# MechaCritter/Python-Visual-Similarity

Measured on AMD Instinct MI355X. Metric: images/sec encoded + top-k retrieved, VLAD K256 RootSIFT, higher is better.
Workload: dtype f32

## Files before the change

include/pvsim.h:

```cpp
#ifndef PVSIM_H
#define PVSIM_H

#include <stddef.h>
#include <stdint.h>

#ifdef __cplusplus
extern "C" {
#endif

#define PVS_VERSION 103

typedef enum {
  PVS_OK = 0,
  PVS_ERR_INVALID = 1,
  PVS_ERR_NO_DEVICE = 2,
  PVS_ERR_OOM = 3,
  PVS_ERR_UNSUPPORTED = 4,
  PVS_ERR_DIM = 5,
  PVS_ERR_CAPACITY = 6
} pvs_status;

typedef enum {
  PVS_DESC_F32 = 0,
  PVS_DESC_F32_ROOTSIFT = 1,
  PVS_DESC_U8_ROOTSIFT = 2
} pvs_desc_kind;

typedef enum {
  PVS_OPT_ASSIGN_PREFILTER = 0,
  PVS_OPT_VLAD_PATH = 1,
  PVS_OPT_TOPK_SELECT_ONLY = 2,
  PVS_OPT_AGG_VARIANT = 3,
  PVS_OPT_FISHER_SCALE = 4,
  PVS_OPT_COUNT_ = 5
} pvs_option;

typedef struct pvs_ctx pvs_ctx;
typedef struct pvs_codebook pvs_codebook;
typedef struct pvs_gmm pvs_gmm;
typedef struct pvs_pca pvs_pca;
typedef struct pvs_comm pvs_comm;

typedef struct {
  double power_norm_weight;
  double norm_order;
  double epsilon;
} pvs_norm_params;

int pvs_version(void);
const char* pvs_last_error(void);
int pvs_device_count(int* count);
int pvs_init(int device_id, void* stream, pvs_ctx** out);
int pvs_destroy(pvs_ctx* ctx);
int pvs_sync(pvs_ctx* ctx);
void* pvs_stream(pvs_ctx* ctx);
int pvs_device_name(pvs_ctx* ctx, char* buf, size_t buflen);
int pvs_set_option(pvs_ctx* ctx, int option, int value);
int pvs_get_option(pvs_ctx* ctx, int option, int* value);

int pvs_malloc(pvs_ctx* ctx, size_t bytes, void** dptr);
int pvs_free(pvs_ctx* ctx, void* dptr);
int pvs_memcpy_h2d(pvs_ctx* ctx, void* dst_dev, const void* src_host, size_t bytes);
int pvs_memcpy_d2h(pvs_ctx* ctx, void* dst_host, const void* src_dev, size_t bytes);
int pvs_memset(pvs_ctx* ctx, void* dst_dev, int value, size_t bytes);

int pvs_fill_dev(pvs_ctx* ctx, void* dst_dev, int64_t n_elems, int elem_bytes, uint64_t pattern);
int pvs_stream_wait(pvs_ctx* waiter, pvs_ctx* signal);

int pvs_codebook_create(pvs_ctx* ctx, const float* centroids , int K, int D, pvs_codebook** out);
int pvs_codebook_destroy(pvs_ctx* ctx, pvs_codebook* cb);
int pvs_gmm_create(pvs_ctx* ctx, const double* weights , const double* means ,
                   const double* covariances , int K, int D, pvs_gmm** out);
int pvs_gmm_destroy(pvs_ctx* ctx, pvs_gmm* g);
int pvs_pca_create(pvs_ctx* ctx, const float* components , const float* mean ,
                   int n_components, int d_in, pvs_pca** out);
int pvs_pca_destroy(pvs_ctx* ctx, pvs_pca* p);

int pvs_vlad_encode(pvs_ctx* ctx, const pvs_codebook* cb, const pvs_pca* pca, const void* desc,
                    int desc_kind, const int64_t* offsets, int64_t n_images, const pvs_norm_params* prm,
                    float* out, int32_t* out_labels);
int pvs_vlad_encode_dev(pvs_ctx* ctx, const pvs_codebook* cb, const pvs_pca* pca, const void* d_desc,
                        int desc_kind, const int64_t* d_offsets, int64_t n_images, int64_t total_desc,
                        const pvs_norm_params* prm, float* d_out, int32_t* d_labels, float* d_inv_norm);
int pvs_kmeans_predict_dev(pvs_ctx* ctx, const pvs_codebook* cb, const void* d_desc, int desc_kind,
                           int64_t total_desc, int32_t* d_labels);

int pvs_fisher_encode(pvs_ctx* ctx, const pvs_gmm* g, const pvs_pca* pca, const void* desc, int desc_kind,
// ... 154 lines not shown
```

python-visual-similarity_amd/csrc/assign_prefilter.hpp:

```cpp
#pragma once

#include "common.hpp"
#include "desc_load.hpp"

namespace pvs {

typedef _Float16 f16x8_t __attribute__((ext_vector_type(8)));
typedef _Float16 f16x4_t __attribute__((ext_vector_type(4)));

constexpr int ASSIGN_THREADS = 512;
constexpr int ASSIGN_ROWS = (ASSIGN_THREADS / 64) * 32;

struct Assign16Args {
  const void* X;
  int64_t total;
  int D, ld;
  const _Float16* C16;
  const float* cnorm;
  int K_pad, D_pad16;
  int c_shift;
  float cmax;
  const _Float16* cnk;
  int cn_e1, K;
  int32_t* labels;
  int64_t* amb_rows;
  unsigned long long* amb_count;
  int64_t cap;
  float2* rowstat;
  unsigned long long* stamps;
  int nprod;
  int shape16;
};

int launch_assign16x(pvs_ctx* ctx, const Assign16Args& p, int kind, size_t lds, int grid);

__device__ __forceinline__ void pf_fill_sqrt_table(uint32_t* lds_t) {
  if (threadIdx.x < 256) {
    const float sv = sqrtf((float)threadIdx.x);
    const _Float16 hi = (_Float16)sv, lo = (_Float16)(sv - (float)hi);
    lds_t[threadIdx.x] = (uint32_t)__builtin_bit_cast(unsigned short, hi) | ((uint32_t)__builtin_bit_cast(unsigned short, lo) << 16);
  }
}
__device__ __forceinline__ void pf_u8_fragment(const uint32_t* lds_t, const uint32_t* xw, f16x8_t* xh, f16x8_t* xl) {
  uint32_t hw[4], lw[4];
#pragma unroll
  for (int i = 0; i < 2; ++i)
#pragma unroll
    for (int pq = 0; pq < 2; ++pq) {
      const uint32_t w = xw[i];
      const uint32_t e0 = lds_t[(w >> (16 * pq)) & 0xffu], e1 = lds_t[(w >> (16 * pq + 8)) & 0xffu];
      hw[2 * i + pq] = __builtin_amdgcn_perm(e1, e0, 0x05040100u);
      lw[2 * i + pq] = __builtin_amdgcn_perm(e1, e0, 0x07060302u);
    }
  *xh = __builtin_bit_cast(f16x8_t, make_uint4(hw[0], hw[1], hw[2], hw[3]));
  *xl = __builtin_bit_cast(f16x8_t, make_uint4(lw[0], lw[1], lw[2], lw[3]));
}

template <int KIND, int NP, bool LUT>
__device__ __forceinline__ float prefilter_eps(float nx, float cmax, float lut_sd, float sqrt_d) {
  const float xc = nx * cmax;
  constexpr float conv_err = DescTraits<KIND>::rootsift ? 4.8e-7f : 0.f;
  const float cc = LUT ? cmax * cmax * lut_sd : cmax * cmax;
  constexpr float drop_err = (3 - NP) * 4.9e-4f;
  return 2.f * (4.8e-7f + 2.4e-7f + 4.8e-5f + 7.7e-6f + 1e-9f + conv_err + drop_err) * xc * (1.f + sqrt_d * 1e-9f) + (LUT ? 6.0e-7f : 2.4e-7f) * (cc + 2.f * xc);
}

__device__ __forceinline__ void pf_label_or_list(const Assign16Args& a, bool settled, bool leader, int64_t row, int bidx, int lane,
                                                 unsigned int* s_count, int64_t* my_rows) {
  const bool amb = leader && !settled;
  const unsigned long long amask = __ballot(amb);
  unsigned int base = 0;
  if (amask != 0ull) {
    if (lane == 0) base = atomicAdd(s_count, (unsigned int)__popcll(amask));
    base = __shfl(base, 0, 64);
  }
  if (leader) {
    if (settled) a.labels[row] = bidx;
    else my_rows[base + __popcll(amask & ((1ull << lane) - 1ull))] = row;
  }
}

}
```

python-visual-similarity_amd/csrc/common.hpp:

```cpp
#pragma once
#include <hip/hip_runtime.h>

#include <cmath>
#include <cstdarg>
#include <cstdint>
#include <cstdio>
#include <cstring>
#include <map>
#include <type_traits>
#include <vector>

#include "../../include/pvsim.h"
#include "../../include/pvsim_diag.h"
#include "workspace.hpp"

#define PVS_EXPORT extern "C" __attribute__((visibility("default")))

namespace pvs {

void set_error(const char* fmt, ...);

#define PVS_FAIL(code, ...)        \
  do {                             \
    ::pvs::set_error(__VA_ARGS__); \
    return (code);                 \
  } while (0)

#define PVS_HIP(expr)                                                                    \
  do {                                                                                   \
    hipError_t e__ = (expr);                                                             \
    if (e__ != hipSuccess) {                                                             \
      ::pvs::set_error("%s failed: %s (%s:%d)", #expr, hipGetErrorString(e__), __FILE__, \
                       __LINE__);                                                        \
      return e__ == hipErrorOutOfMemory ? PVS_ERR_OOM : PVS_ERR_NO_DEVICE;               \
    }                                                                                    \
  } while (0)

#define PVS_TRY(expr)                 \
  do {                                \
    int s__ = (expr);                 \
    if (s__ != PVS_OK) return s__;    \
  } while (0)

constexpr int WAVE = 64;

enum TimerSlot { T_ASSIGN = 0, T_AGGREGATE = 1, T_GEMM = 2, T_TOPK = 3, T_FPOST = 4, T_FMOM = 5, T_MISC = 6, T_RESCORE = 7 };

struct TimerRec {
  hipEvent_t a, b;
  int slot;
};

}

struct pvs_ctx {
  int device = 0;
  hipStream_t stream = nullptr;
  bool owns_stream = false;
  int num_cu = 256;
  static constexpr int NWS = 17;
  void* ws[NWS] = {};
  size_t ws_bytes[NWS] = {};
  struct GemmPlanSlot {
    int key[4] = {-1, -1, -1, -1};
    int n_main = 0, n_tail = 0, splitk = 1;
    void* d_tiles = nullptr;
    size_t cap = 0;
  } gemm_plan[5];
  std::map<const void*, int> lds_attr;
  int opt[PVS_OPT_COUNT_] = {1, 0, 0, 0, 0};
  unsigned int* d_queue = nullptr;
  unsigned long long* d_fused_stamps = nullptr;
  bool timers_on = false;
  std::vector<pvs::TimerRec> pending;
  std::vector<hipEvent_t> event_pool;
  std::multimap<size_t, void*> block_cache;
  std::map<void*, size_t> block_size;
  size_t block_cache_bytes = 0;
  void* h_stage = nullptr;
  size_t h_stage_bytes = 0;
  static constexpr int DSIFT_RING = 4;
  void* dsift_h[DSIFT_RING] = {};
  size_t dsift_h_bytes[DSIFT_RING] = {};
  hipEvent_t dsift_ev[DSIFT_RING] = {};
  int dsift_next = 0;
  double t_total[PVS_TIMER_SLOTS] = {0};
  int64_t t_count[PVS_TIMER_SLOTS] = {0};
};

struct pvs_codebook {
  int K = 0, D = 0;
  int K_pad = 0, D_pad = 0;
  float* d_cent = nullptr;
  float* d_cpad = nullptr;
  float* d_cnorm = nullptr;
  void* d_c16 = nullptr;
  int D_pad16 = 0;
  int c16_shift = 0;
  float cmax = 0.f;
  void* d_cnk = nullptr;
  void* d_c16n = nullptr;
  int cn_e1 = 0;
};

struct pvs_gmm {
  int K = 0, D = 0;
  double* d_w = nullptr;
  double* d_mu = nullptr;
  double* d_cov = nullptr;
  double* d_prec = nullptr;
  double* d_mup = nullptr;
  double* d_inv_mu = nullptr;
  double* d_inv_sg = nullptr;
  double* d_const = nullptr;
};

struct pvs_pca {
  int C = 0, Din = 0;
  float* d_comp = nullptr;
  float* d_off = nullptr;
};

namespace pvs {
// ... 131 lines not shown
```

python-visual-similarity_amd/csrc/vlad.hip:

```cpp
#include "assign_prefilter.hpp"

namespace pvs {

typedef float f32x16 __attribute__((ext_vector_type(16)));

struct AssignArgs {
  const void* X;
  int64_t total;
  int D, ld;
  const float* Cpad;
  const float* cnorm;
  int K_pad, D_pad;
  int32_t* labels;
  const int64_t* rows;
  const unsigned long long* nrows;
  int64_t rows_cap;
};

constexpr int ASSIGN_DCHUNK = 128;

template <int NT, int KIND, bool VEC>
__global__ __launch_bounds__(ASSIGN_THREADS, 2) void assign_kernel(AssignArgs a) {
  extern __shared__ __attribute__((aligned(16))) char smem[];
  constexpr int CB = 32 * NT;
  const int cw_max = a.D_pad < ASSIGN_DCHUNK ? a.D_pad : ASSIGN_DCHUNK;
  const int stride = cw_max + 4;
  float* lds_c = reinterpret_cast<float*>(smem);
  float* lds_n = lds_c + CB * stride;

  const int lane = threadIdx.x & 63, wave = threadIdx.x >> 6;
  const int j = lane & 31, h = lane >> 5;
  const int ncb = a.K_pad / CB;
  const int nsc = (a.D_pad + ASSIGN_DCHUNK - 1) / ASSIGN_DCHUNK;
  const bool restage = (ncb * nsc) > 1;
  const int64_t n_items = a.rows ? (int64_t)a.nrows[blockIdx.x] : a.total;
  const int64_t nblocks = (n_items + ASSIGN_ROWS - 1) / ASSIGN_ROWS;
  const int64_t* const my_rows = a.rows ? a.rows + (int64_t)blockIdx.x * a.rows_cap : nullptr;

  auto stage = [&](int cb, int sc) {
    const int cw = min(ASSIGN_DCHUNK, a.D_pad - sc * ASSIGN_DCHUNK);
    const int c4n = cw >> 2;
    for (int idx = threadIdx.x; idx < CB * c4n; idx += ASSIGN_THREADS) {
      const int r = idx / c4n, c4 = idx - r * c4n;
      const float4 v = *reinterpret_cast<const float4*>(a.Cpad + (int64_t)(cb * CB + r) * a.D_pad +
                                                        sc * ASSIGN_DCHUNK + 4 * c4);
      *reinterpret_cast<float4*>(lds_c + r * stride + 4 * c4) = v;
    }
    for (int idx = threadIdx.x; idx < CB; idx += ASSIGN_THREADS) lds_n[idx] = a.cnorm[cb * CB + idx];
  };

  if (!restage) {
    stage(0, 0);
    __syncthreads();
  }

  for (int64_t blk = my_rows ? 0 : blockIdx.x; blk < nblocks; blk += my_rows ? 1 : gridDim.x) {
    const int64_t item = blk * ASSIGN_ROWS + wave * 32 + j;
    const bool rvalid = item < n_items;
    const int64_t row = (my_rows && rvalid) ? my_rows[item] : item;
    float best = INFINITY;
    int bidx = 0;

    for (int cb = 0; cb < ncb; ++cb) {
      f32x16 acc[NT];
#pragma unroll
      for (int t = 0; t < NT; ++t)
#pragma unroll
        for (int r = 0; r < 16; ++r) acc[t][r] = 0.f;

      for (int sc = 0; sc < nsc; ++sc) {
        if (restage) {
          __syncthreads();
          stage(cb, sc);
          __syncthreads();
        }
        const int dc = sc * ASSIGN_DCHUNK;
        const int nt = min(ASSIGN_DCHUNK, a.D_pad - dc) >> 3;

        float4 xb[16];
#pragma unroll
        for (int t = 0; t < 16; ++t) {
          xb[t] = make_float4(0.f, 0.f, 0.f, 0.f);
          if (t < nt) {
            const int d = dc + 8 * t + 4 * h;
            if constexpr (VEC) {
              if (rvalid && d < a.D) xb[t] = load4<KIND>(a.X, row, a.ld, d);
            } else {
              if (rvalid) {
// ... 406 lines not shown
    }
  }
  __syncthreads();
  if (threadIdx.x == 0) a.amb_count[blockIdx.x] = s_count;
}

template <int NT, int KIND>
static int launch_assign_nt(pvs_ctx* ctx, const AssignArgs& a, bool vec, size_t lds, int grid) {
  auto kv = assign_kernel<NT, KIND, true>;
  auto ks = assign_kernel<NT, KIND, false>;
  return launch_lds(ctx, vec ? kv : ks, dim3(grid), dim3(ASSIGN_THREADS), lds, a);
}

template <int KIND>
static int launch_assign_kind(pvs_ctx* ctx, const AssignArgs& a, int nt, bool vec, size_t lds, int grid) {
  switch (nt) {
    case 8: return launch_assign_nt<8, KIND>(ctx, a, vec, lds, grid);
    case 4: return launch_assign_nt<4, KIND>(ctx, a, vec, lds, grid);
    case 2: return launch_assign_nt<2, KIND>(ctx, a, vec, lds, grid);
    default: return launch_assign_nt<1, KIND>(ctx, a, vec, lds, grid);
  }
}

template <int NT, int KIND>
static int launch_assign16_nt(pvs_ctx* ctx, const Assign16Args& p, bool vec, size_t lds, int grid) {
  auto kv = assign16_kernel<NT, KIND, true, 0>;
  auto ks = assign16_kernel<NT, KIND, false, 0>;
  auto k8 = assign16_kernel<NT, KIND, true, 8>;
  auto k = vec ? (p.D == 128 && p.D_pad16 == 128 ? k8 : kv) : ks;
  if constexpr (NT == 8) {
    if (k == k8 && p.nprod == 3 && p.shape16 && p.stamps == nullptr) return launch_assign16x(ctx, p, KIND, lds, grid);
  }
  if constexpr (NT == 8) {
    if (k == k8 && p.nprod == 2) k = assign16_kernel<NT, KIND, true, 8, false, 2>;
    if (k == k8 && p.nprod == 1) k = assign16_kernel<NT, KIND, true, 8, false, 1>;
  }
  if constexpr (NT == 8) {
    if (p.stamps != nullptr && k == k8) k = assign16_kernel<NT, KIND, true, 8, true>;
  }
  return launch_lds(ctx, k, dim3(grid), dim3(ASSIGN_THREADS), lds, p);
}
template <int KIND>
static int launch_assign16_kind(pvs_ctx* ctx, const Assign16Args& p, int nt, bool vec, size_t lds, int grid) {
  switch (nt) {
    case 8: return launch_assign16_nt<8, KIND>(ctx, p, vec, lds, grid);
    case 4: return launch_assign16_nt<4, KIND>(ctx, p, vec, lds, grid);
    case 2: return launch_assign16_nt<2, KIND>(ctx, p, vec, lds, grid);
    case 1: return launch_assign16_nt<1, KIND>(ctx, p, vec, lds, grid);
    default: PVS_FAIL(PVS_ERR_INVALID, "assignment prefilter: unexpected table padding");
  }
}
static int launch_assign16(pvs_ctx* ctx, const Assign16Args& p, int kind, int nt, bool vec, size_t lds, int grid) {
  return dispatch_desc_kind(kind, [&](auto k) { return launch_assign16_kind<decltype(k)::value>(ctx, p, nt, vec, lds, grid); });
}

int assign_tiles_for(int K) {
  const int k32 = (K + 31) / 32 * 32;
  return k32 > 128 ? 8 : (k32 > 64 ? 4 : (k32 > 32 ? 2 : 1));
}

int launch_assign(pvs_ctx* ctx, const pvs_codebook* cb, const void* d_desc, int kind, int64_t total, int ld,
                  int32_t* d_labels, const float2** rowstat_out) {
  if (rowstat_out) *rowstat_out = nullptr;
  if (total <= 0) return PVS_OK;
  const bool rs = kind != PVS_DESC_F32;
  if (rs && cb->D > ASSIGN_DCHUNK)
    PVS_FAIL(PVS_ERR_UNSUPPORTED, "fused RootSIFT needs D <= %d (got %d)", ASSIGN_DCHUNK, cb->D);
  const int nt = assign_tiles_for(cb->K);
  if (cb->K_pad % (32 * nt) != 0) PVS_FAIL(PVS_ERR_INVALID, "codebook padding does not match the tile count");
  AssignArgs a{d_desc, total, cb->D, ld, cb->d_cpad, cb->d_cnorm, cb->K_pad, cb->D_pad, d_labels, nullptr, nullptr, 0};
  const int esz = kind == PVS_DESC_U8_ROOTSIFT ? 1 : 4;
  const bool vec = (cb->D % 4 == 0) && (ld % 4 == 0) && ((reinterpret_cast<uintptr_t>(d_desc) % (4 * esz)) == 0);
  const int cw = cb->D_pad < ASSIGN_DCHUNK ? cb->D_pad : ASSIGN_DCHUNK;
  const size_t lds = (size_t)(32 * nt) * (cw + 4) * 4 + (size_t)(32 * nt) * 4;
  const int64_t nblocks = (total + ASSIGN_ROWS - 1) / ASSIGN_ROWS;
  const int grid = (int)(nblocks < ctx->num_cu ? nblocks : ctx->num_cu);
  ScopedTimer tm(ctx, T_ASSIGN);
  const bool pre = cb->d_c16 != nullptr && total >= 4096 && ctx->opt[PVS_OPT_ASSIGN_PREFILTER] != 0;
  if (pre) {
    const int64_t cap = (nblocks + grid - 1) / grid * ASSIGN_ROWS;
    char* ws = nullptr;
    const bool stat = rowstat_out != nullptr && kind == PVS_DESC_U8_ROOTSIFT;
    WsLayout<> lay;
    const auto cnt_p = lay.add<unsigned long long>((size_t)grid);
    const auto rows_p = lay.add<int64_t>((size_t)grid * cap);
    const auto stat_p = lay.add<float2>(stat ? (size_t)total : 0);
    PVS_TRY(ws_reserve(ctx, WS_LISTS, lay.bytes(), &ws));
    unsigned long long* cnt = cnt_p(ws);
    int64_t* rows = rows_p(ws);
    float2* rowstat = stat ? stat_p(ws) : nullptr;
    if (stat) *rowstat_out = rowstat;
    Assign16Args p{d_desc, total, cb->D, ld, static_cast<const _Float16*>(cb->d_c16), cb->d_cnorm, cb->K_pad, cb->D_pad16,
                   cb->c16_shift, cb->cmax, static_cast<const _Float16*>(cb->d_cnk), cb->cn_e1, cb->K, d_labels, rows, cnt, cap, rowstat,
                   ctx->d_fused_stamps, ctx->opt[PVS_OPT_ASSIGN_PREFILTER] == 2 ? 2 : (ctx->opt[PVS_OPT_ASSIGN_PREFILTER] == 3 ? 1 : 3),
                   ctx->opt[PVS_OPT_ASSIGN_PREFILTER] == 4 ? 1 : 0};
    const size_t lds16 = (size_t)2 * cb->K_pad * (128 + 8) * 2 + (size_t)cb->K_pad * 4 + (size_t)cb->K_pad * 8 + 1024;
    PVS_TRY(launch_assign16(ctx, p, kind, cb->K_pad / 32, vec, lds16, grid));
    a.rows = rows;
    a.nrows = cnt;
    a.rows_cap = cap;
  }
  return dispatch_desc_kind(kind, [&](auto k) { return launch_assign_kind<decltype(k)::value>(ctx, a, nt, vec, lds, grid); });
}

struct AggArgs {
  const void* X;
  int D, ld;
  const int64_t* offsets;
  const int32_t* labels;
  const float* cent;
  int K;
  float power, eps;
  int norm_mode;
  float norm_p;
  float* out;
  float* inv_norm;
  const float2* rowstat;
};

constexpr int AGG_THREADS = 256;
constexpr int AGG_WAVES = AGG_THREADS / 64;
constexpr int AGG_CHUNK = 4096;

template <int KIND, int GROUP, int VW, int NREG, bool HIOCC = false>
__global__ __launch_bounds__(AGG_THREADS, (HIOCC ? 8 : 1)) void vlad_aggregate_kernel(AggArgs a) {
  extern __shared__ __attribute__((aligned(16))) char smem[];
  const int K = a.K, D = a.D;
  int* hist = reinterpret_cast<int*>(smem);
  int* start = hist + AGG_WAVES * K;
  float* rowsq = reinterpret_cast<float*>(start + K + 1);
  int* scan_tmp = reinterpret_cast<int*>(rowsq + K);
  uint16_t* order = reinterpret_cast<uint16_t*>(scan_tmp + AGG_WAVES);

  const int img = blockIdx.x;
  const int tid = threadIdx.x, lane = tid & 63, wave = tid >> 6;
  const int64_t row0 = a.offsets[img];
  const int64_t n = a.offsets[img + 1] - row0;
  float* out_img = a.out + (int64_t)img * K * D;

  constexpr int NGROUPS = AGG_THREADS / GROUP;
  const int grp = tid / GROUP, gl = tid % GROUP;
  int kbits = 0;
  while ((1 << kbits) < K) ++kbits;

  const int64_t nchunks = n > 0 ? (n + AGG_CHUNK - 1) / AGG_CHUNK : 1;
  for (int64_t ch = 0; ch < nchunks; ++ch) {
    const int64_t cbase = row0 + ch * AGG_CHUNK;
    const int cn = (int)min((int64_t)AGG_CHUNK, n - ch * AGG_CHUNK);
    const bool last = (ch == nchunks - 1);

    for (int i = tid; i < AGG_WAVES * K; i += AGG_THREADS) hist[i] = 0;
    __syncthreads();
    const int per_wave = (cn + AGG_WAVES - 1) / AGG_WAVES;
// ... 467 lines not shown
```

python-visual-similarity_amd/csrc/vlad_fused.hip:

```cpp
#include "common.hpp"
#include "desc_load.hpp"

namespace pvs {

typedef float f32x16 __attribute__((ext_vector_type(16)));
typedef _Float16 f16x8_t __attribute__((ext_vector_type(8)));
typedef _Float16 f16x4_t __attribute__((ext_vector_type(4)));

constexpr int FU_THREADS = 512;
constexpr int FU_R = 64;
constexpr int FU_XS = 132;
constexpr int FU_TS = 1056;
constexpr int FU_TILE = 8 * FU_TS;
constexpr int FU_UNUSABLE = 0x7fffffff;
constexpr int FU_KB = 4;

constexpr int FU_OFF_X32 = 0;
constexpr int FU_OFF_XH = FU_OFF_X32 + FU_R * FU_XS * 4;
constexpr int FU_OFF_XL = FU_OFF_XH + 2 * FU_TILE;
constexpr int FU_OFF_NX = FU_OFF_XL + 2 * FU_TILE;
constexpr int FU_OFF_XSH = FU_OFF_NX + 256;
constexpr int FU_OFF_CAND = FU_OFF_XSH + 256;
constexpr int FU_OFF_ENT = FU_OFF_CAND + 8 * FU_R * 8;
constexpr int FU_OFF_ENTV = FU_OFF_ENT + 2048;
constexpr int FU_OFF_ROWSQ = FU_OFF_ENTV + 4096;
constexpr int FU_OFF_MISC = FU_OFF_ROWSQ + 1024;
constexpr int FU_LDS = FU_OFF_MISC + 64;

struct FusedArgs {
  const void* X;
  int ld;
  const int64_t* offsets;
  int64_t n_images;
  const _Float16* c16n;
  const _Float16* cnk;
  const float* cnorm;
  const float* cent;
  const float* cpad;
  int K, c_shift, cn_e1;
  float cmax;
  float power, eps;
  int norm_mode;
  float norm_p;
  float* out;
  float* inv_norm;
  int32_t* labels;
  unsigned int* queue;
  unsigned long long* stamps;
};

template <int KIND>
struct FuStage {
  float4 v[4];
};
// ... 240 lines not shown
        const float margin = usable ? (eps_a * s_nx[lane] + eps_b) * ldexpf(1.f, a.c_shift + xsh) : 0.f;
        const bool settled = usable && label < a.K && (t1 - t2 > margin);
        const float thr = t1 - margin;
        const unsigned long long umask = __ballot(rvalid && !settled);
        FU_STAMP(2)
        if constexpr (DIAG) { dg_c[0] += 1; dg_c[3] += __popcll(umask); }
        if (umask != 0ull) {
          int cm = 0, am = 0;
          if (rvalid && !settled) {
            if (!usable || label >= a.K) {
              cm = 0xff; am = 0xff;
            } else {
#pragma unroll
              for (int w = 0; w < 8; ++w) {
                const float2 c = s_cand[w * FU_R + lane];
                if (c.x >= thr) cm |= 1 << w;
                if (c.y >= thr) am |= 1 << w;
              }
            }
          }
          const int ne = __popc(cm);
          int incl = ne;
#pragma unroll
          for (int d = 1; d < 64; d <<= 1) {
            const int o = __shfl_up(incl, d, 64);
            if (lane >= d) incl += o;
          }
          const int ebase = incl - ne;
          const int E = __shfl(incl, 63, 64);
          if constexpr (DIAG) { dg_c[1] += 1; dg_c[2] += E; }
          if (wave == 0 && ne > 0) {
            int e = ebase;
            for (int w = 0; w < 8; ++w)
              if (cm & (1 << w)) {
                const int sidx = 31 - (__float_as_int(s_cand[w * FU_R + lane].x) & 31);
                s_ent[e++] = lane | (w << 8) | (((am >> w) & 1) << 12) | (sidx << 16);
              }
          }
          __syncthreads();
          for (int e0 = 0; e0 < E; e0 += 16) {
            const int e = e0 + 2 * wave + h;
            const bool elive = e < E;
            const int ent = elive ? s_ent[e] : 0;
            const int er = ent & 0xff, ew = (ent >> 8) & 7, eall = (ent >> 12) & 1, esi = (ent >> 16) & 31;
            const int k = 32 * ew + (eall ? j : esi);
            const bool active = elive && (eall || j == 0);
            const float* xr = x32 + er * FU_XS;
            const float* cr = a.cpad + (size_t)k * 128;
            float dot = 0.f;
#pragma unroll 2
            for (int b8 = 0; b8 < 128; b8 += 8) {
              const float4 xa = *reinterpret_cast<const float4*>(xr + b8), xb = *reinterpret_cast<const float4*>(xr + b8 + 4);
              const float4 ca = *reinterpret_cast<const float4*>(cr + b8), cb = *reinterpret_cast<const float4*>(cr + b8 + 4);
              dot = fmaf(ca.x, xa.x, dot); dot = fmaf(cb.x, xb.x, dot);
              dot = fmaf(ca.y, xa.y, dot); dot = fmaf(cb.y, xb.y, dot);
              dot = fmaf(ca.z, xa.z, dot); dot = fmaf(cb.z, xb.z, dot);
              dot = fmaf(ca.w, xa.w, dot); dot = fmaf(cb.w, xb.w, dot);
            }
            const float v = fmaf(-2.f, dot, a.cnorm[k]);
            const bool ok = active && (v < INFINITY);
            float vv = ok ? v : INFINITY;
            int kk = ok ? k : 0x7fffffff;
#pragma unroll
            for (int m = 16; m >= 1; m >>= 1) {
              const float ov = __shfl_xor(vv, m, 64);
              const int okk = __shfl_xor(kk, m, 64);
              const bool take = ov < vv || (ov == vv && okk < kk);
              vv = take ? ov : vv;
              kk = take ? okk : kk;
            }
            if (elive && j == 0) s_entv[e] = make_float2(vv, __int_as_float(kk));
          }
          __syncthreads();
          if (rvalid && !settled) {
            float bv = INFINITY;
            int bk = 0x7fffffff;
            for (int i = 0; i < ne; ++i) {
              const float2 r = s_entv[ebase + i];
              const int rk = __float_as_int(r.y);
              if (r.x < bv || (r.x == bv && rk < bk)) { bv = r.x; bk = rk; }
            }
            label = bv < INFINITY ? bk : 0;
          }
        }
        FU_STAMP(3)
        if (a.labels != nullptr && wave == 0 && rvalid) a.labels[sbase + lane] = label;

        unsigned long long mine = __ballot(rvalid && (label >> 5) == wave);
        while (mine != 0ull) {
          int rr[FU_KB], ll[FU_KB];
          int cntb = 0;
#pragma unroll
          for (int u = 0; u < FU_KB; ++u) {
            const bool live = mine != 0ull;
            const int r = live ? (int)__builtin_ctzll(mine) : 0;
            if (live) { mine &= mine - 1ull; ++cntb; }
            rr[u] = r;
            ll[u] = __builtin_amdgcn_readlane(label, r);
          }
          float2 xv[FU_KB], cv[FU_KB];
#pragma unroll
          for (int u = 0; u < FU_KB; ++u) {
            xv[u] = *reinterpret_cast<const float2*>(x32 + rr[u] * FU_XS + 2 * lane);
            cv[u] = *reinterpret_cast<const float2*>(a.cent + (size_t)ll[u] * 128 + 2 * lane);
          }
#pragma unroll
          for (int u = 0; u < FU_KB; ++u) {
            if (u < cntb) {
              const float dx = xv[u].x - cv[u].x, dy = xv[u].y - cv[u].y;
#define FU_ADD(c) case c: acc[2 * c] += dx; acc[2 * c + 1] += dy; break;
// ... 124 lines not shown
```

python-visual-similarity_amd/pvsim/_ffi.py:

```python
from __future__ import annotations

import ctypes as C
import os
import threading

import numpy as np

from ._errors import CapacityError

_HERE = os.path.dirname(os.path.abspath(__file__))
LIB_PATH = os.environ.get("PVSIM_LIB", os.path.join(_HERE, "libpvsim_hip.so"))

PVS_OK, PVS_ERR_INVALID, PVS_ERR_NO_DEVICE, PVS_ERR_OOM, PVS_ERR_UNSUPPORTED, PVS_ERR_DIM, PVS_ERR_CAPACITY = range(7)
_EXC = {PVS_ERR_INVALID: ValueError, PVS_ERR_NO_DEVICE: RuntimeError, PVS_ERR_OOM: MemoryError,
        PVS_ERR_UNSUPPORTED: NotImplementedError, PVS_ERR_DIM: RuntimeError, PVS_ERR_CAPACITY: CapacityError}

DESC_F32, DESC_F32_ROOTSIFT, DESC_U8_ROOTSIFT = 0, 1, 2
OPT_ASSIGN_PREFILTER, OPT_VLAD_PATH, OPT_TOPK_SELECT_ONLY, OPT_AGG_VARIANT, OPT_FISHER_SCALE = 0, 1, 2, 3, 4
PIX_U8_RGB, PIX_U8_GRAY, PIX_F32_RGB, PIX_F32_GRAY = 0, 1, 2, 3
DSIFT_U8, DSIFT_F32, DSIFT_F32_RAW, DSIFT_F32_QUANT = 0, 1, 2, 3
COMBINE_CHUNK_BYTES, COMBINE_BATCH = 8192, 8
VLAD_PATH_AUTO, VLAD_PATH_GATHER, VLAD_PATH_STREAM, VLAD_PATH_FUSED = 0, 1, 2, 3
TIMER_NAMES = ("assign", "aggregate", "cosine_gemm", "topk", "fisher_posterior", "fisher_moments", "misc", "rescore")


class NormParams(C.Structure):
    _fields_ = [("power_norm_weight", C.c_double), ("norm_order", C.c_double), ("epsilon", C.c_double)]


_vp, _i64, _int, _sz = C.c_void_p, C.c_int64, C.c_int, C.c_size_t
_pp = C.POINTER(C.c_void_p)
_np = C.POINTER(NormParams)

SIGNATURES = {
    "pvs_version": [],
    "pvs_last_error": [],
    "pvs_device_count": [C.POINTER(C.c_int)],
    "pvs_init": [_int, _vp, _pp],
    "pvs_destroy": [_vp],
    "pvs_sync": [_vp],
    "pvs_stream": [_vp],
    "pvs_device_name": [_vp, C.c_char_p, _sz],
    "pvs_set_option": [_vp, _int, _int],
    "pvs_get_option": [_vp, _int, C.POINTER(C.c_int)],
    "pvs_malloc": [_vp, _sz, _pp],
    "pvs_free": [_vp, _vp],
    "pvs_memcpy_h2d": [_vp, _vp, _vp, _sz],
    "pvs_memcpy_d2h": [_vp, _vp, _vp, _sz],
    "pvs_memset": [_vp, _vp, _int, _sz],
    "pvs_fill_dev": [_vp, _vp, _i64, _int, C.c_uint64],
    "pvs_stream_wait": [_vp, _vp],
    "pvs_comm_unique_id": [_vp],
    "pvs_comm_init": [_vp, _int, _int, _vp, _pp],
    "pvs_comm_destroy": [_vp],
    "pvs_comm_library": [],
    "pvs_allgather_dev": [_vp, _vp, _vp, _sz],
    "pvs_alltoall_dev": [_vp, _vp, _vp, _sz],
    "pvs_sendrecv_dev": [_vp, _int, _vp, _vp, _vp, _vp, _vp],
    "pvs_allreduce_max_f64": [_vp, _vp, _int],
    "pvs_comm_barrier": [_vp],
    "pvs_codebook_create": [_vp, _vp, _int, _int, _pp],
    "pvs_codebook_destroy": [_vp, _vp],
    "pvs_gmm_create": [_vp, _vp, _vp, _vp, _int, _int, _pp],
    "pvs_gmm_destroy": [_vp, _vp],
    "pvs_pca_create": [_vp, _vp, _vp, _int, _int, _pp],
    "pvs_pca_destroy": [_vp, _vp],
    "pvs_vlad_encode": [_vp, _vp, _vp, _vp, _int, _vp, _i64, _np, _vp, _vp],
    "pvs_vlad_encode_dev": [_vp, _vp, _vp, _vp, _int, _vp, _i64, _i64, _np, _vp, _vp, _vp],
    "pvs_kmeans_predict_dev": [_vp, _vp, _vp, _int, _i64, _vp],
    "pvs_fisher_encode": [_vp, _vp, _vp, _vp, _int, _vp, _i64, _np, _vp],
    "pvs_fisher_encode_dev": [_vp, _vp, _vp, _vp, _int, _vp, _i64, _i64, _np, _vp, _int],
# ... 131 lines not shown
```

Baseline: 416,900.

## Add near-candidate pass to resolve ambiguous assignment rows before full exact assign

New measurement: 418,700, median of 6. About the same (+0.4%).

```diff
diff --git a/include/pvsim.h b/include/pvsim.h
--- a/include/pvsim.h
+++ b/include/pvsim.h
@@ -32,7 +32,8 @@
   PVS_OPT_TOPK_SELECT_ONLY = 2,
   PVS_OPT_AGG_VARIANT = 3,
   PVS_OPT_FISHER_SCALE = 4,
-  PVS_OPT_COUNT_ = 5
+  PVS_OPT_ASSIGN_NEAR = 5,
+  PVS_OPT_COUNT_ = 6
 } pvs_option;
 
 typedef struct pvs_ctx pvs_ctx;
diff --git a/python-visual-similarity_amd/csrc/assign_prefilter.hpp b/python-visual-similarity_amd/csrc/assign_prefilter.hpp
--- a/python-visual-similarity_amd/csrc/assign_prefilter.hpp
+++ b/python-visual-similarity_amd/csrc/assign_prefilter.hpp
@@ -65,6 +65,101 @@
   return 2.f * (4.8e-7f + 2.4e-7f + 4.8e-5f + 7.7e-6f + 1e-9f + conv_err + drop_err) * xc * (1.f + sqrt_d * 1e-9f) + (LUT ? 6.0e-7f : 2.4e-7f) * (cc + 2.f * xc);
 }
 
+template <int KIND>
+struct PfRow {
+  f16x8_t xh[8], xl[8];
+  float nx;
+  float lut_sd = 1.f;
+  _Float16 lut_f1 = (_Float16)0.f, lut_f2 = (_Float16)0.f;
+  int x_shift = 0;
+  bool finite;
+};
+template <int KIND>
+__device__ __forceinline__ void pf_row_front(const Assign16Args& a, int64_t r, int h, const uint32_t* lds_t, PfRow<KIND>& o) {
+  constexpr bool LUT = KIND == PVS_DESC_U8_ROOTSIFT;
+  if constexpr (LUT) {
+    uint32_t xw[8][2];
+    const uint8_t* pr = static_cast<const uint8_t*>(a.X) + r * a.ld + 4 * h;
+#pragma unroll
+    for (int t = 0; t < 8; ++t) {
+      xw[t][0] = *reinterpret_cast<const uint32_t*>(pr + 16 * t);
+      xw[t][1] = *reinterpret_cast<const uint32_t*>(pr + 16 * t + 8);
+    }
+    unsigned ssum = 0;
+#pragma unroll
+    for (int t = 0; t < 8; ++t) {
+      ssum = __builtin_amdgcn_sad_u8(xw[t][0], 0u, ssum);
+      ssum = __builtin_amdgcn_sad_u8(xw[t][1], 0u, ssum);
+    }
+    ssum += __shfl_xor(ssum, 32, 64);
+    const float sf = (float)ssum, dd = sf + 1e-7f;
+    o.lut_sd = sqrtf(dd);
+    const float ff = ldexpf(o.lut_sd, a.cn_e1);
+    o.lut_f1 = (_Float16)ff;
+    o.lut_f2 = (_Float16)(ff - (float)o.lut_f1);
+    o.finite = ff >= 0.125f && ff <= 32768.f;
+    o.nx = sqrtf(sf) * 1.0001f;
+#pragma unroll
+    for (int t = 0; t < 8; ++t) pf_u8_fragment(lds_t, xw[t], &o.xh[t], &o.xl[t]);
+  } else {
+    float xf[8][8];
+#pragma unroll
+    for (int t = 0; t < 8; ++t) {
+      const float4 v0 = load4<KIND>(a.X, r, a.ld, 16 * t + 4 * h);
+      const float4 v1 = load4<KIND>(a.X, r, a.ld, 16 * t + 4 * h + 8);
+      xf[t][0] = v0.x; xf[t][1] = v0.y; xf[t][2] = v0.z; xf[t][3] = v0.w;
+      xf[t][4] = v1.x; xf[t][5] = v1.y; xf[t][6] = v1.z; xf[t][7] = v1.w;
+    }
+    float n2 = 0.f, amax = 0.f, rs_r = 0.f;
+    if constexpr (DescTraits<KIND>::rootsift) {
+      float s = 0.f, rmax = 0.f;
+#pragma unroll
+      for (int t = 0; t < 8; ++t)
+#pragma unroll
+        for (int q = 0; q < 8; ++q) {
+          s += xf[t][q];
+          rmax = fmaxf(rmax, xf[t][q]);
+        }
+      s += __shfl_xor(s, 32, 64);
+      rmax = fmaxf(rmax, __shfl_xor(rmax, 32, 64));
+      rs_r = 1.0f / (s + 1e-7f);
+      n2 = s * rs_r * 1.0001f;
+      amax = __builtin_amdgcn_sqrtf(rmax * rs_r) * 1.0001f;
+      if (!(s >= 0.f) || !(rmax * rs_r <= 3.0e38f)) n2 = NAN;
+    } else {
+#pragma unroll
+      for (int t = 0; t < 8; ++t)
+#pragma unroll
+        for (int q = 0; q < 8; ++q) {
+          n2 = fmaf(xf[t][q], xf[t][q], n2);
+          amax = fmaxf(amax, fabsf(xf[t][q]));
+        }
+      n2 += __shfl_xor(n2, 32, 64);
+      amax = fmaxf(amax, __shfl_xor(amax, 32, 64));
+    }
+    o.nx = sqrtf(n2) * 1.0001f;
+    int ex = 13;
+    if (amax > 0.f) (void)frexpf(amax, &ex);
+    o.x_shift = 13 - ex;
+    o.finite = o.nx <= 3.0e38f;
+    if (o.x_shift > 40 || o.x_shift < -40) { o.finite = false; o.x_shift = 0; }
+    if (o.x_shift + a.cn_e1 < -14 || o.x_shift + a.cn_e1 > 15) o.finite = false;
+    const float xs = ldexpf(1.f, o.x_shift);
+    const float rs_rs = rs_r * xs * xs;
+#pragma unroll
+    for (int t = 0; t < 8; ++t)
+#pragma unroll
+      for (int q = 0; q < 8; ++q) {
+        float v;
+        if constexpr (DescTraits<KIND>::rootsift) v = __builtin_amdgcn_sqrtf(xf[t][q] * rs_rs);
+        else v = xf[t][q] * xs;
+        const _Float16 hi = (_Float16)v;
+        o.xh[t][q] = hi;
+        o.xl[t][q] = (_Float16)(v - (float)hi);
+      }
+  }
+}
+
 __device__ __forceinline__ void pf_label_or_list(const Assign16Args& a, bool settled, bool leader, int64_t row, int bidx, int lane,
                                                  unsigned int* s_count, int64_t* my_rows) {
   const bool amb = leader && !settled;
diff --git a/python-visual-similarity_amd/csrc/common.hpp b/python-visual-similarity_amd/csrc/common.hpp
--- a/python-visual-similarity_amd/csrc/common.hpp
+++ b/python-visual-similarity_amd/csrc/common.hpp
@@ -68,7 +68,7 @@
     size_t cap = 0;
   } gemm_plan[5];
   std::map<const void*, int> lds_attr;
-  int opt[PVS_OPT_COUNT_] = {1, 0, 0, 0, 0};
+  int opt[PVS_OPT_COUNT_] = {1, 0, 0, 0, 0, 0};
   unsigned int* d_queue = nullptr;
   unsigned long long* d_fused_stamps = nullptr;
   bool timers_on = false;
diff --git a/python-visual-similarity_amd/csrc/exact_dot.hpp b/python-visual-similarity_amd/csrc/exact_dot.hpp
--- /dev/null
+++ b/python-visual-similarity_amd/csrc/exact_dot.hpp
@@ -0,0 +1,15 @@
+#pragma once
+
+#include "common.hpp"
+
+namespace pvs {
+
+__device__ __forceinline__ float exact_dot_step8(const float4 ca, const float4 cb, const float4 xa, const float4 xb, float dot) {
+  dot = fmaf(ca.x, xa.x, dot); dot = fmaf(cb.x, xb.x, dot);
+  dot = fmaf(ca.y, xa.y, dot); dot = fmaf(cb.y, xb.y, dot);
+  dot = fmaf(ca.z, xa.z, dot); dot = fmaf(cb.z, xb.z, dot);
+  dot = fmaf(ca.w, xa.w, dot); dot = fmaf(cb.w, xb.w, dot);
+  return dot;
+}
+
+}
diff --git a/python-visual-similarity_amd/csrc/vlad.hip b/python-visual-similarity_amd/csrc/vlad.hip
--- a/python-visual-similarity_amd/csrc/vlad.hip
+++ b/python-visual-similarity_amd/csrc/vlad.hip
@@ -1,4 +1,5 @@
 #include "assign_prefilter.hpp"
+#include "exact_dot.hpp"
 
 namespace pvs {
 
@@ -34,6 +35,7 @@
   const int nsc = (a.D_pad + ASSIGN_DCHUNK - 1) / ASSIGN_DCHUNK;
   const bool restage = (ncb * nsc) > 1;
   const int64_t n_items = a.rows ? (int64_t)a.nrows[blockIdx.x] : a.total;
+  if (a.rows && n_items == 0) return;
   const int64_t nblocks = (n_items + ASSIGN_ROWS - 1) / ASSIGN_ROWS;
   const int64_t* const my_rows = a.rows ? a.rows + (int64_t)blockIdx.x * a.rows_cap : nullptr;
 
@@ -546,6 +548,267 @@
 }
 static int launch_assign16(pvs_ctx* ctx, const Assign16Args& p, int kind, int nt, bool vec, size_t lds, int grid) {
   return dispatch_desc_kind(kind, [&](auto k) { return launch_assign16_kind<decltype(k)::value>(ctx, p, nt, vec, lds, grid); });
+}
+
+constexpr int NEAR_SLOTS = 7;
+
+struct AssignNearArgs {
+  Assign16Args p;
+  const float* Cpad;
+  unsigned long long* cand;
+  int64_t* ovf_rows;
+  unsigned long long* ovf_count;
+  unsigned long long* stats;
+};
+
+constexpr int NEAR_CSTRIDE = 132;
+constexpr size_t NEAR_LDS1 = (size_t)2 * 256 * (128 + 8) * 2 + 256 * 8 + 1024 + (size_t)NEAR_SLOTS * ASSIGN_THREADS * 4;
+constexpr size_t NEAR_LDS2 = (size_t)256 * NEAR_CSTRIDE * 4 + 256 * 4;
+constexpr size_t NEAR_LDS = NEAR_LDS1 > NEAR_LDS2 ? NEAR_LDS1 : NEAR_LDS2;
+
+template <int KIND>
+__global__ __launch_bounds__(ASSIGN_THREADS, 2) void assign_near_kernel(AssignNearArgs a) {
+  extern __shared__ __attribute__((aligned(16))) char smem[];
+  __shared__ unsigned int s_ovf, s_stat[2];
+  const Assign16Args& p = a.p;
+  const int64_t n_items = (int64_t)p.amb_count[blockIdx.x];
+  if (n_items == 0) {
+    if (threadIdx.x == 0) a.ovf_count[blockIdx.x] = 0ull;
+    return;
+  }
+  constexpr bool LUT = KIND == PVS_DESC_U8_ROOTSIFT;
+  constexpr int stride = 128 + 8;
+  _Float16* lds_h = reinterpret_cast<_Float16*>(smem);
+  _Float16* lds_l = lds_h + 256 * stride;
+  _Float16* lds_k = lds_l + 256 * stride;
+  uint32_t* lds_t = reinterpret_cast<uint32_t*>(lds_k + 4 * 256);
+  float* lds_v = reinterpret_cast<float*>(lds_t + 256);
+  const int lane = threadIdx.x & 63, wave = threadIdx.x >> 6;
+  const int j = lane & 31, h = lane >> 5;
+  const int64_t nblocks = (n_items + ASSIGN_ROWS - 1) / ASSIGN_ROWS;
+  const int64_t* const my_rows = p.amb_rows + (int64_t)blockIdx.x * p.cap;
+  unsigned long long* const my_cand = a.cand + (int64_t)blockIdx.x * p.cap;
+  int64_t* const my_ovf = a.ovf_rows + (int64_t)blockIdx.x * p.cap;
+
+  for (int idx = threadIdx.x; idx < 2 * 256 * 16; idx += ASSIGN_THREADS) {
+    const int r = idx >> 4, c8 = idx & 15;
+    *reinterpret_cast<uint4*>(lds_h + r * stride + 8 * c8) = *reinterpret_cast<const uint4*>(p.C16 + (int64_t)r * 128 + 8 * c8);
+  }
+  for (int idx = threadIdx.x; idx < 256; idx += ASSIGN_THREADS)
+    *reinterpret_cast<uint2*>(lds_k + 4 * idx) = *reinterpret_cast<const uint2*>(p.cnk + 4 * idx);
+  if constexpr (LUT) pf_fill_sqrt_table(lds_t);
+  if (threadIdx.x == 0) { s_ovf = 0u; s_stat[0] = 0u; s_stat[1] = 0u; }
+  __syncthreads();
+  const float sqrt_d = sqrtf((float)p.D);
+
+  for (int64_t blk = 0; blk < nblocks; ++blk) {
+    const int64_t item = blk * ASSIGN_ROWS + wave * 32 + j;
+    const bool rvalid = item < n_items;
+    const int64_t row = my_rows[rvalid ? item : n_items - 1];
+    PfRow<KIND> x;
+    pf_row_front<KIND>(p, row, h, lds_t, x);
+    f16x8_t cnb;
+    {
+      const _Float16 pw = (h == 0 && x.finite) ? (_Float16)ldexpf(1.f, x.x_shift + p.cn_e1) : (_Float16)0.f;
+#pragma unroll
+      for (int q = 0; q < 8; ++q) cnb[q] = (_Float16)0.f;
+      if constexpr (LUT) {
+        if (h == 0 && x.finite) { cnb[0] = x.lut_f1; cnb[1] = x.lut_f2; cnb[2] = x.lut_f1; cnb[3] = x.lut_f2; cnb[4] = x.lut_f1; cnb[5] = x.lut_f2; }
+      } else {
+        cnb[0] = pw; cnb[1] = pw; cnb[2] = pw;
+      }
+    }
+    const float m2s = -2.f * ldexpf(1.f, -(x.x_shift + p.c_shift));
+    const float eps2 = 2.f * prefilter_eps<KIND, 3, LUT>(x.nx, p.cmax, x.lut_sd, sqrt_d);
+    float smax = -INFINITY;
+    unsigned long long rpk = 0ull;
+    int rcnt = 0;
+#pragma unroll
+    for (int g = 0; g < 4; ++g) {
+      f32x16 acc[2];
+#pragma unroll
+      for (int u = 0; u < 2; ++u)
+#pragma unroll
+        for (int r = 0; r < 16; ++r) acc[u][r] = 0.f;
+#pragma unroll
+      for (int t = 0; t < 8; ++t) {
+        f16x8_t fh[2], fl[2];
+#pragma unroll
+        for (int u = 0; u < 2; ++u) {
+          fh[u] = *reinterpret_cast<const f16x8_t*>(lds_h + (32 * (2 * g + u) + j) * stride + 16 * t + 8 * h);
+          fl[u] = *reinterpret_cast<const f16x8_t*>(lds_l + (32 * (2 * g + u) + j) * stride + 16 * t + 8 * h);
+        }
+        __builtin_amdgcn_sched_barrier(0);
+#pragma unroll
+        for (int u = 0; u < 2; ++u) acc[u] = __builtin_amdgcn_mfma_f32_32x32x16_f16(fl[u], x.xh[t], acc[u], 0, 0, 0);
+#pragma unroll
+        for (int u = 0; u < 2; ++u) acc[u] = __builtin_amdgcn_mfma_f32_32x32x16_f16(fh[u], x.xl[t], acc[u], 0, 0, 0);
+#pragma unroll
+        for (int u = 0; u < 2; ++u) acc[u] = __builtin_amdgcn_mfma_f32_32x32x16_f16(fh[u], x.xh[t], acc[u], 0, 0, 0);
+        __builtin_amdgcn_sched_barrier(0);
+      }
+#pragma unroll
+      for (int u = 0; u < 2; ++u) {
+        const f16x4_t ck = *reinterpret_cast<const f16x4_t*>(lds_k + 4 * (32 * (2 * g + u) + j));
+        f16x8_t ca;
+#pragma unroll
+        for (int q = 0; q < 8; ++q) ca[q] = (_Float16)0.f;
+        if constexpr (LUT) {
+          if (h == 0) { ca[0] = ck[0]; ca[1] = ck[0]; ca[2] = ck[1]; ca[3] = ck[1]; ca[4] = ck[2]; ca[5] = ck[2]; }
+        } else {
+          if (h == 0) { ca[0] = ck[0]; ca[1] = ck[1]; ca[2] = ck[2]; }
+        }
+        acc[u] = __builtin_amdgcn_mfma_f32_32x32x16_f16(ca, cnb, acc[u], 0, 0, 0);
+      }
+      float gm = -INFINITY;
+#pragma unroll
+      for (int u = 0; u < 2; ++u)
+#pragma unroll
+        for (int r = 0; r < 16; ++r) gm = fmaxf(gm, acc[u][r]);
+      gm = fmaxf(gm, __shfl_xor(gm, 32, 64));
+      smax = fmaxf(smax, gm);
+      const float vthr_g = smax * m2s + eps2;
+#pragma unroll
+      for (int u = 0; u < 2; ++u)
+#pragma unroll
+        for (int r = 0; r < 16; ++r) {
+          const unsigned long long kc = (unsigned long long)(32 * (2 * g + u) + 8 * (r >> 2) + (r & 3));
+          const float sv = acc[u][r];
+          if (sv * m2s <= vthr_g) {
+            if (rcnt < NEAR_SLOTS) {
+              rpk |= kc << (8 * rcnt);
+              lds_v[rcnt * ASSIGN_THREADS + threadIdx.x] = sv;
+            }
+            ++rcnt;
+          }
+        }
+    }
+    const float best = smax * m2s;
+    const float vthr = best + eps2;
+    unsigned long long pk = 0ull;
+    int cnt = 0;
+    bool padded = rcnt > NEAR_SLOTS;
+#pragma unroll
+    for (int i = 0; i < NEAR_SLOTS; ++i) {
+      if (i < rcnt) {
+        const float sv = lds_v[i * ASSIGN_THREADS + threadIdx.x];
+        if (sv * m2s <= vthr) {
+          const int k = (int)((rpk >> (8 * i)) & 0xffull) + 4 * h;
+          pk |= (unsigned long long)k << (8 * cnt);
+          ++cnt;
+          padded = padded || k >= p.K;
+        }
+      }
+    }
+    const int ocnt = __shfl_xor(cnt, 32, 64);
+    const unsigned long long opk = __shfl_xor(pk, 32, 64);
+    padded = padded || (__shfl_xor((int)padded, 32, 64) != 0);
+    const int total = cnt + ocnt;
+    const bool usable = x.finite && fabsf(best) <= 3.0e38f && !padded && total >= 1 && total <= NEAR_SLOTS;
+    const bool leader = h == 0 && rvalid;
+    const bool ovf = leader && !usable;
+    const unsigned long long omask = __ballot(ovf);
+    unsigned int obase = 0;
+    if (omask != 0ull) {
+      if (lane == 0) obase = atomicAdd(&s_ovf, (unsigned int)__popcll(omask));
+      obase = __shfl(obase, 0, 64);
+    }
+    if (leader) {
+      unsigned long long word = 0ull;
+      if (usable) word = ((unsigned long long)total << 56) | pk | (opk << (8 * cnt));
+      else my_ovf[obase + __popcll(omask & ((1ull << lane) - 1ull))] = row;
+      my_cand[item] = word;
+    }
+    if (a.stats != nullptr) {
+      const unsigned long long umask = __ballot(leader && usable);
+      int tc = (leader && usable) ? total : 0;
+      for (int m = 32; m >= 1; m >>= 1) tc += __shfl_xor(tc, m, 64);
+      if (lane == 0) { atomicAdd(&s_stat[0], (unsigned int)__popcll(umask)); atomicAdd(&s_stat[1], (unsigned int)tc); }
+    }
+  }
+  __syncthreads();
+  if (threadIdx.x == 0) {
+    a.ovf_count[blockIdx.x] = s_ovf;
+    if (a.stats != nullptr) {
+      atomicAdd(a.stats + 12, (unsigned long long)n_items);
+      atomicAdd(a.stats + 13, (unsigned long long)s_stat[0]);
+      atomicAdd(a.stats + 14, (unsigned long long)s_ovf);
+      atomicAdd(a.stats + 15, (unsigned long long)s_stat[1]);
+    }
+  }
+
+  float* lds_c = reinterpret_cast<float*>(smem);
+  float* lds_cn = lds_c + 256 * NEAR_CSTRIDE;
+  for (int idx = threadIdx.x; idx < 256 * 32; idx += ASSIGN_THREADS) {
+    const int r = idx >> 5, c4 = idx & 31;
+    *reinterpret_cast<float4*>(lds_c + r * NEAR_CSTRIDE + 4 * c4) = *reinterpret_cast<const float4*>(a.Cpad + (int64_t)r * 128 + 4 * c4);
+  }
+  for (int idx = threadIdx.x; idx < 256; idx += ASSIGN_THREADS) lds_cn[idx] = p.cnorm[idx];
+  __syncthreads();
+
+  for (int64_t blk = 0; blk < nblocks; ++blk) {
+    const int64_t item = blk * ASSIGN_ROWS + wave * 32 + j;
+    const bool rvalid = item < n_items;
+    unsigned long long word = rvalid ? my_cand[item] : 0ull;
+    word = __shfl(word, j, 64);
+    const int cnt = (int)(word >> 56);
+    if (__ballot(cnt > 0) == 0ull) continue;
+    const int64_t row = my_rows[rvalid ? item : n_items - 1];
+    float4 xm[16];
+#pragma unroll
+    for (int t = 0; t < 16; ++t) xm[t] = load4<KIND>(p.X, row, p.ld, 8 * t + 4 * h);
+    if constexpr (DescTraits<KIND>::rootsift) {
+      float s = 0.f;
+#pragma unroll
+      for (int t = 0; t < 16; ++t) s += (xm[t].x + xm[t].y) + (xm[t].z + xm[t].w);
+      s += __shfl_xor(s, 32, 64);
+      const RootsiftRow<KIND> rr(s);
+#pragma unroll
+      for (int t = 0; t < 16; ++t) {
+        xm[t].x = rr(xm[t].x);
+        xm[t].y = rr(xm[t].y);
+        xm[t].z = rr(xm[t].z);
+        xm[t].w = rr(xm[t].w);
+      }
+    }
+    float4 xa[16], xb[16];
+#pragma unroll
+    for (int t = 0; t < 16; ++t) {
+      float4 o;
+      o.x = __shfl_xor(xm[t].x, 32, 64);
+      o.y = __shfl_xor(xm[t].y, 32, 64);
+      o.z = __shfl_xor(xm[t].z, 32, 64);
+      o.w = __shfl_xor(xm[t].w, 32, 64);
+      xa[t] = h == 0 ? xm[t] : o;
+      xb[t] = h == 0 ? o : xm[t];
+      __builtin_amdgcn_sched_barrier(0);
+    }
+    float bv = INFINITY;
+    int bk = 0x7fffffff;
+    for (int i = h; __ballot(i < cnt) != 0ull; i += 2) {
+      const int k = i < cnt ? (int)((word >> (8 * i)) & 0xffull) : 0;
+      const float* cr = lds_c + k * NEAR_CSTRIDE;
+      float dot = 0.f;
+#pragma unroll
+      for (int t = 0; t < 16; ++t) {
+        const float4 ca = *reinterpret_cast<const float4*>(cr + 8 * t), cb = *reinterpret_cast<const float4*>(cr + 8 * t + 4);
+        dot = exact_dot_step8(ca, cb, xa[t], xb[t], dot);
+        if ((t & 3) == 3) __builtin_amdgcn_sched_barrier(0);
+      }
+      const float v = fmaf(-2.f, dot, lds_cn[k]);
+      const bool ok = i < cnt && v < INFINITY;
+      if (ok && (v < bv || (v == bv && k < bk))) { bv = v; bk = k; }
+    }
+    const float ov = __shfl_xor(bv, 32, 64);
+    const int ok2 = __shfl_xor(bk, 32, 64);
+    if (ov < bv || (ov == bv && ok2 < bk)) { bv = ov; bk = ok2; }
+    if (h == 0 && cnt > 0) p.labels[row] = bv < INFINITY ? bk : 0;
+  }
+}
+
+template <int KIND>
+static int launch_assign_near_kind(pvs_ctx* ctx, const AssignNearArgs& a, int grid) {
+  return launch_lds(ctx, assign_near_kernel<KIND>, dim3(grid), dim3(ASSIGN_THREADS), NEAR_LDS, a);
 }
 
 int assign_tiles_for(int K) {
@@ -579,6 +842,9 @@
     const auto cnt_p = lay.add<unsigned long long>((size_t)grid);
     const auto rows_p = lay.add<int64_t>((size_t)grid * cap);
     const auto stat_p = lay.add<float2>(stat ? (size_t)total : 0);
+    const auto cand_p = lay.add<unsigned long long>((size_t)grid * cap);
+    const auto ovf_p = lay.add<int64_t>((size_t)grid * cap);
+    const auto ovfc_p = lay.add<unsigned long long>((size_t)grid);
     PVS_TRY(ws_reserve(ctx, WS_LISTS, lay.bytes(), &ws));
     unsigned long long* cnt = cnt_p(ws);
     int64_t* rows = rows_p(ws);
@@ -593,6 +859,14 @@
     a.rows = rows;
     a.nrows = cnt;
     a.rows_cap = cap;
+    const bool near = ctx->opt[PVS_OPT_ASSIGN_NEAR] == 0 && ctx->opt[PVS_OPT_ASSIGN_PREFILTER] == 1 && vec && cb->D == 128 &&
+                      cb->D_pad == 128 && cb->D_pad16 == 128 && cb->K_pad == 256;
+    if (near) {
+      AssignNearArgs na{p, cb->d_cpad, cand_p(ws), ovf_p(ws), ovfc_p(ws), ctx->d_fused_stamps};
+      PVS_TRY(dispatch_desc_kind(kind, [&](auto k) { return launch_assign_near_kind<decltype(k)::value>(ctx, na, grid); }));
+      a.rows = na.ovf_rows;
+      a.nrows = na.ovf_count;
+    }
   }
   return dispatch_desc_kind(kind, [&](auto k) { return launch_assign_kind<decltype(k)::value>(ctx, a, nt, vec, lds, grid); });
 }
diff --git a/python-visual-similarity_amd/csrc/vlad_fused.hip b/python-visual-similarity_amd/csrc/vlad_fused.hip
--- a/python-visual-similarity_amd/csrc/vlad_fused.hip
+++ b/python-visual-similarity_amd/csrc/vlad_fused.hip
@@ -1,5 +1,6 @@
 #include "common.hpp"
 #include "desc_load.hpp"
+#include "exact_dot.hpp"
 
 namespace pvs {
 
@@ -346,10 +347,7 @@
             for (int b8 = 0; b8 < 128; b8 += 8) {
               const float4 xa = *reinterpret_cast<const float4*>(xr + b8), xb = *reinterpret_cast<const float4*>(xr + b8 + 4);
               const float4 ca = *reinterpret_cast<const float4*>(cr + b8), cb = *reinterpret_cast<const float4*>(cr + b8 + 4);
-              dot = fmaf(ca.x, xa.x, dot); dot = fmaf(cb.x, xb.x, dot);
-              dot = fmaf(ca.y, xa.y, dot); dot = fmaf(cb.y, xb.y, dot);
-              dot = fmaf(ca.z, xa.z, dot); dot = fmaf(cb.z, xb.z, dot);
-              dot = fmaf(ca.w, xa.w, dot); dot = fmaf(cb.w, xb.w, dot);
+              dot = exact_dot_step8(ca, cb, xa, xb, dot);
             }
             const float v = fmaf(-2.f, dot, a.cnorm[k]);
             const bool ok = active && (v < INFINITY);
diff --git a/python-visual-similarity_amd/pvsim/_ffi.py b/python-visual-similarity_amd/pvsim/_ffi.py
--- a/python-visual-similarity_amd/pvsim/_ffi.py
+++ b/python-visual-similarity_amd/pvsim/_ffi.py
@@ -16,7 +16,7 @@
         PVS_ERR_UNSUPPORTED: NotImplementedError, PVS_ERR_DIM: RuntimeError, PVS_ERR_CAPACITY: CapacityError}
 
 DESC_F32, DESC_F32_ROOTSIFT, DESC_U8_ROOTSIFT = 0, 1, 2
-OPT_ASSIGN_PREFILTER, OPT_VLAD_PATH, OPT_TOPK_SELECT_ONLY, OPT_AGG_VARIANT, OPT_FISHER_SCALE = 0, 1, 2, 3, 4
+OPT_ASSIGN_PREFILTER, OPT_VLAD_PATH, OPT_TOPK_SELECT_ONLY, OPT_AGG_VARIANT, OPT_FISHER_SCALE, OPT_ASSIGN_NEAR = 0, 1, 2, 3, 4, 5
 PIX_U8_RGB, PIX_U8_GRAY, PIX_F32_RGB, PIX_F32_GRAY = 0, 1, 2, 3
 DSIFT_U8, DSIFT_F32, DSIFT_F32_RAW, DSIFT_F32_QUANT = 0, 1, 2, 3
 COMBINE_CHUNK_BYTES, COMBINE_BATCH = 8192, 8
```
